# facebookresearch/vggsfm

Hardware: NVIDIA H100
Metric: BA iterations/sec (higher is better)
Workload: dtype f64

## Files before the change

vggsfm_b200/csrc/ba_lm.h:

```cpp
#pragma once
#include <math.h>
#include <stddef.h>
#include "common.cuh"

namespace vgg {

enum : int {
  SCAL_CAM_QUAD = 0, SCAL_CAM_STEP2 = 1, SCAL_PT_QUAD = 2, SCAL_PT_STEP2 = 3, SCAL_GMAX_C = 4, SCAL_GMAX_P = 5,
  SCAL_PT_FAIL = 6, SCAL_CAM_BAD = 7, SCAL_XNORM_C = 8, SCAL_DOUBLES = 16,
};
enum : int {
  SMALL_COST = 0, SMALL_PT_QUAD = 1, SMALL_PT_STEP2 = 2, SMALL_PT_FAIL = 3, SMALL_GMAX_P = 4, SMALL_XNORM_P = 5,
  SMALL_MODEL_CHANGE = 6, SMALL_VEC = 8,
};
enum : int { INFO_CHOL = 0, INFO_TRSV = 1, INFO_FABRIC = 2, INFO_INTS = 4 };

struct LmRecord {
  double scal[8], small[8], chol_info, trsv_info, xnorm_c, fabric_timeout, cg[5];
  double cost() const { return small[SMALL_COST]; }
  double gmax() const {
    return isnan(scal[SCAL_GMAX_C]) || isnan(scal[SCAL_GMAX_P]) ? NAN : fmax(scal[SCAL_GMAX_C], scal[SCAL_GMAX_P]);
  }
};
#define VGG_REC(field) ((int)(offsetof(LmRecord, field) / sizeof(double)))
enum : int { REC_DOUBLES = 24, REC_DOUBLES_CG = 28, REC_CAP = 32 };

struct Reduced {
  double *S, *rhs, *hdiag, *gvec;
};
inline size_t reduced_doubles(int D, int Dpad) { return (size_t)D * Dpad + 3 * (size_t)Dpad; }
// ... 19 lines not shown
```

vggsfm_b200/csrc/ba_schur.cu:

```cuda
#include <stddef.h>
#include <algorithm>
#include <vector>
#include "ba_lm.h"
#include "ba_obs.h"
#include "common.cuh"
#include "dev_probes.h"
#include "syrk_work.h"

namespace vgg {

__device__ __forceinline__ void ar_add(double* local, double* mc, double v) {
  if (mc) asm volatile("multimem.red.relaxed.sys.global.add.f64 [%0], %1;" ::"l"(mc), "d"(v) : "memory");
  else atomicAdd(local, v);
}
__device__ __forceinline__ void ar_put(double* local, double* mc, double v) {
  if (mc) asm volatile("multimem.red.relaxed.sys.global.add.f64 [%0], %1;" ::"l"(mc), "d"(v) : "memory");
  else *local = v;
}

__global__ void jacobi_scale_points_kernel(int N, const double* __restrict__ H_pp, double* __restrict__ sc_p, int enable) {
  const int n = blockIdx.x * blockDim.x + threadIdx.x;
  if (n >= N) return;
  const double* h = H_pp + (size_t)n * 6;
  sc_p[n * 3 + 0] = enable ? 1.0 / (1.0 + sqrt(h[0])) : 1.0;
// ... 323 lines not shown
    for (int mt = 0; mt < 4; ++mt)
#pragma unroll
      for (int nt = 0; nt < 4; ++nt)
#pragma unroll
        for (int h = 0; h < 4; ++h) {
          const int r = wk.bi * SF_BM + wm * 64 + mt * 16 + g + 8 * (h >> 1);
          const int col = wk.bj * SF_BM + wn * 32 + nt * 8 + 2 * t + (h & 1);
          syrk_red_upper(Cmat, Dpad, r, col, wk.bj, diag, acc[mt][nt][h], mc_off, fd);
        }
  }
}

__global__ void scale_damp_kernel(int D, int Dpad, double* __restrict__ A, const double* __restrict__ rhs,
                                  const double* __restrict__ hdiag, const double* __restrict__ sc,
                                  const uint8_t* __restrict__ pconst, double radius, double min_diag, double max_diag,
                                  double* __restrict__ bvec) {
  const int j = blockIdx.x * blockDim.x + threadIdx.x;
  const int i = blockIdx.y;
  if (j >= D || j > i) return;
  const bool ci = pconst[i] != 0, cj = pconst[j] != 0;
  double v;
  if (ci || cj) {
    v = (i == j) ? 1.0 : 0.0;
  } else {
    v = A[(size_t)i * Dpad + j] * sc[i] * sc[j];
    if (i == j) v += fmin(fmax(hdiag[i] * sc[i] * sc[i], min_diag), max_diag) / radius;
  }
  A[(size_t)i * Dpad + j] = v;
  if (i == j) {
    const double b = ci ? 0.0 : rhs[i] * sc[i];
    bvec[i] = b;
    A[(size_t)D * Dpad + i] = b;
    if (i == 0) A[(size_t)D * Dpad + D] = 1e300;
  }
}

__global__ void cam_step_kernel(int D, const double* __restrict__ dcs, size_t dcs_stride, const double* __restrict__ sc,
                                const double* __restrict__ hdiag, const double* __restrict__ gvec,
                                const uint8_t* __restrict__ pconst, double radius, double min_diag, double max_diag,
                                double* __restrict__ d_c, double* __restrict__ scal) {
  const int i = blockIdx.x * blockDim.x + threadIdx.x;
  double a = 0, b = 0, bad = 0;
  if (i < D) {
    const double x = pconst[i] ? 0.0 : dcs[(size_t)i * dcs_stride];
    const double dc = x * sc[i];
    d_c[i] = dc;
    if (!isfinite(x)) bad = 1.0;
    const double dcc = fmin(fmax(hdiag[i] * sc[i] * sc[i], min_diag), max_diag);
    a = pconst[i] ? 0.0 : (x * x * dcc / radius - dc * gvec[i]);
    b = dc * dc;
  }
  a = warp_sum(a); b = warp_sum(b); bad = warp_sum(bad);
  if ((threadIdx.x & 31) == 0) {
    atomicAdd(&scal[SCAL_CAM_QUAD], a);
    atomicAdd(&scal[SCAL_CAM_STEP2], b);
    if (bad > 0) atomicAdd(&scal[SCAL_CAM_BAD], bad);
  }
}

constexpr int BS_W = 16;
template <int MODEL, int MODE, bool ROBUST>
__global__ void __launch_bounds__(BS_W * 32) backsub_kernel(
    int S, int N, const float* __restrict__ uv, const uint8_t* __restrict__ mask, const double* __restrict__ poses,
    const double* __restrict__ intr, const double* __restrict__ points, const uint8_t* __restrict__ point_const,
    const double* __restrict__ d_c, double* __restrict__ wacc, const int* __restrict__ fg_tracks, BaLoss loss) {
  using C = BlkCfg<MODEL, MODE>;
  constexpr int DC = C::DC, NS = C::NS;
  __shared__ double s_cam[BS_W][16];
  __shared__ double s_acc[3][BS_W][32];
  const int lane = threadIdx.x & 31, warp = threadIdx.x >> 5, nw = blockDim.x >> 5;
  const int nlo = blockIdx.x * 32, nhi = min(N, nlo + 32);
// ... 73 lines not shown
    const double s0 = sc_p[n * 3], s1 = sc_p[n * 3 + 1], s2 = sc_p[n * 3 + 2];
    const double e0 = d0 / s0, e1 = d1 / s1, e2 = d2 / s2;
    a = pc ? 0.0 : (e0 * e0 * dpp[n * 3] + e1 * e1 * dpp[n * 3 + 1] + e2 * e2 * dpp[n * 3 + 2]) / radius -
                       (d0 * g0 + d1 * g1 + d2 * g2);
    b = pc ? 0.0 : d0 * d0 + d1 * d1 + d2 * d2;
  }
  a = warp_sum(a); b = warp_sum(b);
  if ((threadIdx.x & 31) == 0) {
    atomicAdd(&scal[SCAL_PT_QUAD], a);
    atomicAdd(&scal[SCAL_PT_STEP2], b);
  }
}

__global__ void cam_update_kernel(int S, int dc, int ns, int model, const double* __restrict__ d_c,
                                  const double* __restrict__ poses, const double* __restrict__ intr,
                                  double* __restrict__ poses_c, double* __restrict__ intr_c) {
  const int s = blockIdx.x * blockDim.x + threadIdx.x;
  if (s >= S) return;
  const double* d = d_c + (size_t)s * dc;
  const double p0 = 2.0 * d[0], p1 = 2.0 * d[1], p2 = 2.0 * d[2];
  const double th2 = p0 * p0 + p1 * p1 + p2 * p2;
  const double th = sqrt(th2);
  double a, b;
  if (th < 1e-12) {
    a = 1.0 - th2 / 6.0;
    b = 0.5 - th2 / 24.0;
  } else {
    a = sin(th) / th;
    b = (1.0 - cos(th)) / th2;
  }
  const bool rot = p0 != 0.0 || p1 != 0.0 || p2 != 0.0;
  double E[9];
// ... 11 lines not shown
  Q[7] = d[4] != 0.0 ? P[7] + d[4] : P[7];
  Q[11] = d[5] != 0.0 ? P[11] + d[5] : P[11];
  const int ni = (model == VGG_SIMPLE_PINHOLE) ? 1 : 2;
  double f = intr[s * 4], k = intr[s * 4 + 3];
  const double* di = dc > 6 ? d + 6 : d_c + (size_t)S * dc;
  if (dc > 6 || ns > 0) {
    if (di[0] != 0.0) f += di[0];
    if (ni > 1 && di[1] != 0.0) k += di[1];
  }
  intr_c[s * 4] = f;
  intr_c[s * 4 + 1] = intr[s * 4 + 1];
  intr_c[s * 4 + 2] = intr[s * 4 + 2];
  intr_c[s * 4 + 3] = k;
}

__global__ void extract_gvec_kernel(int S, int dc, int ns, int KR, const double* __restrict__ camrec,
                                    const double* __restrict__ shared_in, double* __restrict__ gvec) {
  const int i = blockIdx.x * blockDim.x + threadIdx.x;
  const int D = S * dc + ns;
  if (i >= D) return;
  gvec[i] = (i < S * dc) ? camrec[(size_t)(i / dc) * KR + (i % dc)] : shared_in[i - S * dc];
}

__global__ void gradmax_kernel(int D, int N, const double* __restrict__ gvec, const uint8_t* __restrict__ pconst,
                               const double* __restrict__ g_p, const uint8_t* __restrict__ point_const,
                               double* __restrict__ scal) {
  const int i = blockIdx.x * blockDim.x + threadIdx.x;
  unsigned long long mc = 0, mp = 0;
  if (i < D && !pconst[i]) mc = (unsigned long long)__double_as_longlong(fabs(gvec[i]));
  if (i < N * 3 && !(point_const && point_const[i / 3])) mp = (unsigned long long)__double_as_longlong(fabs(g_p[i]));
#pragma unroll
  for (int off = 16; off >= 1; off >>= 1) {
    mc = max(mc, __shfl_xor_sync(0xffffffffu, mc, off));
    mp = max(mp, __shfl_xor_sync(0xffffffffu, mp, off));
  }
  if ((threadIdx.x & 31) == 0) {
// ... 75 lines not shown
    if (!work.empty())
      VGG_CUDA_CHECK(cudaMemcpy(hs.work_dev, work.data(), sizeof(SyrkWork) * work.size(), cudaMemcpyHostToDevice));
    hs.nwork = (int)work.size();
    hs.dev = dev;
    hs.Kpad = Kpad;
    hs.Dpad = Dpad;
    hs.ranges = ranges;
  }
  if (hs.nwork == 0) return VGG_OK;
  syrk_f64_kernel<<<std::min(hs.sms, hs.nwork), SF_THREADS, SF_SMEM_BYTES, st>>>(hs.work_dev, hs.nwork, Kpad, Dpad, Zt, Cmat,
                                                                               mc_off, fd);
  VGG_LAUNCH_CHECK();
  return VGG_OK;
}
int launch_scale_damp(int D, int Dpad, double* A, const double* rhs, const double* hdiag, const double* sc,
                      const uint8_t* pconst, double radius, double min_diag, double max_diag, double* bvec,
                      cudaStream_t st) {
  dim3 grid((D + 255) / 256, D);
  scale_damp_kernel<<<grid, 256, 0, st>>>(D, Dpad, A, rhs, hdiag, sc, pconst, radius, min_diag, max_diag, bvec);
  VGG_LAUNCH_CHECK();
  return VGG_OK;
}
int launch_cam_step(int D, const double* dcs, size_t dcs_stride, const double* sc, const double* hdiag, const double* gvec,
                    const uint8_t* pconst, double radius, double min_diag, double max_diag, double* d_c, double* scal,
                    cudaStream_t st) {
  cam_step_kernel<<<(D + 255) / 256, 256, 0, st>>>(D, dcs, dcs_stride, sc, hdiag, gvec, pconst, radius, min_diag, max_diag, d_c, scal);
  VGG_LAUNCH_CHECK();
  return VGG_OK;
}
int launch_backsub(const vgg_ba_problem* p, const double* d_c, double* wacc, const int* fg_tracks, cudaStream_t st) {
  VGG_PICK_BA_KERNEL(kern, backsub_kernel, p);
  const int nw = std::min(BS_W, p->S);
  kern<<<(p->N + 31) / 32, nw * 32, 0, st>>>(p->S, p->N, p->uv, p->mask, p->poses, p->intr, p->points, p->point_const,
                                             d_c, wacc, fg_tracks, ba_loss_of(p));
  VGG_LAUNCH_CHECK();
  return VGG_OK;
}
int launch_point_step(int N, const double* M, const double* g_p, const double* wacc, const double* sc_p,
                      const double* dpp, const uint8_t* point_const, const double* X, double radius, double* Xc,
                      double* scal, cudaStream_t st) {
  point_step_kernel<<<(N + 127) / 128, 128, 0, st>>>(N, M, g_p, wacc, sc_p, dpp, point_const, X, radius, Xc, scal);
  VGG_LAUNCH_CHECK();
  return VGG_OK;
}
int launch_cam_update(int S, int dc, int ns, int model, const double* d_c, const double* poses, const double* intr,
                      double* poses_c, double* intr_c, cudaStream_t st) {
  cam_update_kernel<<<(S + 127) / 128, 128, 0, st>>>(S, dc, ns, model, d_c, poses, intr, poses_c, intr_c);
  VGG_LAUNCH_CHECK();
  return VGG_OK;
}
int launch_extract_gvec(int S, int dc, int ns, int KR, const double* camrec, const double* shared_in, double* gvec,
                        cudaStream_t st) {
  const int D = S * dc + ns;
  extract_gvec_kernel<<<(D + 255) / 256, 256, 0, st>>>(S, dc, ns, KR, camrec, shared_in, gvec);
  VGG_LAUNCH_CHECK();
  return VGG_OK;
}
int launch_gradmax(int D, int N, const double* gvec, const uint8_t* pconst, const double* g_p,
                   const uint8_t* point_const, double* scal, cudaStream_t st) {
  const int n = D > N * 3 ? D : N * 3;
  gradmax_kernel<<<(n + 255) / 256, 256, 0, st>>>(D, N, gvec, pconst, g_p, point_const, scal);
  VGG_LAUNCH_CHECK();
  return VGG_OK;
}

}

extern "C" {

// ... 35 lines not shown
```

vggsfm_b200/csrc/ba_solve.cu:

```cuda
#include <cublas_v2.h>
#include <math.h>
#include <stdlib.h>
#include <string.h>
#include <map>
#include <vector>
#include "ba_lm.h"
#include "ba_pcg.h"
#include "common.cuh"
#include "dev_probes.h"

namespace vgg {

static thread_local char g_err[512] = "";
thread_local long long g_launch_count = 0;
void set_error(const char* fmt, ...) {
  va_list ap;
  va_start(ap, fmt);
  vsnprintf(g_err, sizeof(g_err), fmt, ap);
  va_end(ap);
}

int ba_build_blocks(const vgg_ba_problem* p, double* cost, double* camrec, double* g_p, double* H_pp, double* W,
                    double* shared_out, int tracks_per_warp, const int* fg_tracks, cudaStream_t stream,
                    bool outputs_zeroed = false);
int launch_jacobi_scale_points(int N, const double* H_pp, double* sc_p, int enable, cudaStream_t st);
int launch_jacobi_scale_cams(int D, const double* hdiag, double* sc_c, int enable, cudaStream_t st);
int launch_point_prep(int N, const double* H_pp, const double* g_p, const double* sc_p, const uint8_t* point_const,
                      double radius, double min_diag, double max_diag, double* M, double* q, double* dpp,
                      double* scal, cudaStream_t st);
int launch_assemble_hc(int S, int dc, int ns, int KR, int Dpad, const double* camrec, const double* shared_in,
                       double* Sraw, double* rhs, double* hdiag, double* gvec, ptrdiff_t mc_off, cudaStream_t st);
int launch_z_build(const vgg_ba_problem* p, int Dpad, const double* M, const double* q, double* Zt, double* rhs,
                   ptrdiff_t mc_off, const int* fg_tracks, cudaStream_t st);
int launch_syrk(int Kpad, int Dpad, const double* Zt, double* Cmat, ptrdiff_t mc_off, const std::vector<int>& kb_ranges,
                const FabricDev& fd, cudaStream_t st);
int launch_scale_damp(int D, int Dpad, double* A, const double* rhs, const double* hdiag, const double* sc,
                      const uint8_t* pconst, double radius, double min_diag, double max_diag, double* bvec,
                      cudaStream_t st);
int launch_cam_step(int D, const double* dcs, size_t dcs_stride, const double* sc, const double* hdiag, const double* gvec,
                    const uint8_t* pconst, double radius, double min_diag, double max_diag, double* d_c, double* scal,
                    cudaStream_t st);
int launch_backsub(const vgg_ba_problem* p, const double* d_c, double* wacc, const int* fg_tracks, cudaStream_t st);
int launch_point_step(int N, const double* M, const double* g_p, const double* wacc, const double* sc_p,
                      const double* dpp, const uint8_t* point_const, const double* X, double radius, double* Xc,
                      double* scal, cudaStream_t st);
int launch_cam_update(int S, int dc, int ns, int model, const double* d_c, const double* poses, const double* intr,
                      double* poses_c, double* intr_c, cudaStream_t st);
int launch_extract_gvec(int S, int dc, int ns, int KR, const double* camrec, const double* shared_in, double* gvec,
                        cudaStream_t st);
int launch_gradmax(int D, int N, const double* gvec, const uint8_t* pconst, const double* g_p,
                   const uint8_t* point_const, double* scal, cudaStream_t st);

int launch_trsv_upper(int n, int lda, const double* A, const double* y, size_t y_stride, double* x, long long* stamps,
                      cudaStream_t st);
size_t chol_workspace_doubles(int n);
int chol_lower_inplace(int n, int lda, double* A, double* Ldiag, int* info, const std::vector<int>& end_blk,
                       int arrow_blk, cudaStream_t st);
int launch_fabric_barrier(const FabricDev& fd, size_t flags_off, unsigned long long epoch, int* err, cudaStream_t st);
int launch_fabric_gather(const FabricDev& fd, int nrows, int nmat, int ncols_vec, int lda, cudaStream_t st);
int launch_fabric_allreduce(const FabricDev& fd, size_t flags_off, size_t mail_off, int mail_len, int parity,
                            unsigned long long epoch, double* vec, int count, int max_slot, int* err, cudaStream_t st);

__global__ void pack_scalars_kernel(const double* __restrict__ scal, const double* __restrict__ small,
// ... 646 lines not shown
  const cudaStream_t st = c.ranks.st;
  int rc;
  const size_t off = fab ? (size_t)(it & 1) * fab->lay.arc : 0;
  const Reduced R = reduced_view(fab ? fab->ar_local + off : L.AR, D, L.Dpad);
  const FabricDev fd = fab ? fab->at(off) : FabricDev{};
  if ((rc = schur_build(L, R, pcur, b, c.band, fd, radius, c.opt.min_lm_diagonal, c.opt.max_lm_diagonal, st, fab)))
    return rc;
  if ((rc = fab ? launch_fabric_gather(fd, D + 3, D + 1, D, L.Dpad, st) : c.ranks.sum(R.S, reduced_doubles(D, L.Dpad))))
    return rc;
  if (first && (rc = launch_jacobi_scale_cams(D, R.hdiag, L.sc_c, c.opt.jacobi_scaling, st))) return rc;
  if ((rc = launch_scale_damp(D, L.Dpad, R.S, R.rhs, R.hdiag, L.sc_c, pcur.param_const, radius, c.opt.min_lm_diagonal,
                              c.opt.max_lm_diagonal, L.bvec, st)))
    return rc;
  if ((rc = chol_lower_inplace(D + 1, L.Dpad, R.S, L.chol_diag, L.dev_info + INFO_CHOL, c.band.end_blk, c.band.arrow_blk, st)))
    return rc;
  VGG_CUDA_CHECK(cudaMemsetAsync(L.dev_info + INFO_TRSV, 0, sizeof(int), st));
  *out = LinStep{L.bvec, R.hdiag, R.gvec, 1};
  if (D <= 7000) return launch_trsv_upper(D, L.Dpad, R.S, R.S + D, (size_t)L.Dpad, L.bvec, nullptr, st);
  cublasHandle_t cb = get_cublas();
  if (!cb || cublasSetStream(cb, st) != CUBLAS_STATUS_SUCCESS) {
    set_error("cublasCreate / cublasSetStream failed");
    return VGG_ESOLVER;
  }
  if (cublasDtrsv(cb, CUBLAS_FILL_MODE_LOWER, CUBLAS_OP_T, CUBLAS_DIAG_NON_UNIT, D, R.S, L.Dpad, R.S + D, L.Dpad) !=
      CUBLAS_STATUS_SUCCESS) {
    set_error("cublasDtrsv failed to launch");
    return VGG_ESOLVER;
  }
  g_launch_count += 1;
  *out = LinStep{R.S + D, R.hdiag, R.gvec, (size_t)L.Dpad};
  return VGG_OK;
// ... 18 lines not shown
    op.camrec = B.camrec;
    op.shared_in = B.shared;
  }
  if (first && (rc = launch_jacobi_scale_cams(L.D, B.hdiag, L.sc_c, c.opt.jacobi_scaling, st))) return rc;
  if ((rc = launch_pcg_init(op, B, L.bvec, st)) || (rc = pcg_run(op, lin, B, L.bvec, c.ranks, st))) return rc;
  *out = LinStep{B.x, B.hdiag, B.gvec, 1};
  return VGG_OK;
}

static int reduce_candidate(const LmContext& c, const vgg_ba_problem& pcur, int cur, bool iterative) {
  const Layout& L = c.L;
  const BlockSet& bn = L.blk[cur ^ 1];
  const cudaStream_t st = c.ranks.st;
  const size_t count = SMALL_VEC + (size_t)L.Dpad;
  int rc;
  VGG_CUDA_CHECK(cudaMemsetAsync(L.small, 0, sizeof(double) * count, st));
  if (iterative && (rc = launch_pcg_model_change(&pcur, L.M, L.blk[cur].g_p, L.wacc, L.d_c, c.band.dev.fg_tracks,
                                                 L.small + SMALL_MODEL_CHANGE, st)))
    return rc;
  VGG_CUDA_CHECK(cudaMemcpyAsync(L.small + SMALL_COST, bn.cost, sizeof(double), cudaMemcpyDeviceToDevice, st));
  VGG_CUDA_CHECK(cudaMemcpyAsync(L.small + SMALL_PT_QUAD, L.scal + SCAL_PT_QUAD, sizeof(double) * 2, cudaMemcpyDeviceToDevice, st));
  VGG_CUDA_CHECK(cudaMemcpyAsync(L.small + SMALL_PT_FAIL, L.scal + SCAL_PT_FAIL, sizeof(double), cudaMemcpyDeviceToDevice, st));
  if ((rc = launch_extract_gvec(L.S, L.dc, L.ns, L.KR, bn.camrec, bn.shared, L.small + SMALL_VEC, st))) return rc;
  if (c.opt.parameter_tolerance > 0.0) {
    xnorm_kernel<<<1, 1024, 0, st>>>(L.S, L.N, L.dc, L.ns, pcur.camera_model, pcur.param_const, pcur.point_const,
                                      pcur.poses, pcur.intr, pcur.points, L.scal + SCAL_XNORM_C, L.small + SMALL_XNORM_P);
    VGG_LAUNCH_CHECK();
  }
  return c.ranks.candidate(L.small, count, L.scal, [&] {
    return launch_gradmax(L.D, L.N, L.small + SMALL_VEC, pcur.param_const, bn.g_p, pcur.point_const, L.scal, st);
  });
}

struct LmState {
  double cost, radius, decrease_factor;
  int invalid_steps;
};

// ... 96 lines not shown
  int cur = 0;
  VGG_CUDA_CHECK(cudaMemcpyAsync(L.poses[0], prob->poses, sizeof(double) * (size_t)S * 12, cudaMemcpyDeviceToDevice, st));
  VGG_CUDA_CHECK(cudaMemcpyAsync(L.intr[0], prob->intr, sizeof(double) * (size_t)S * 4, cudaMemcpyDeviceToDevice, st));
  VGG_CUDA_CHECK(cudaMemcpyAsync(L.points[0], prob->points, sizeof(double) * (size_t)N * 3, cudaMemcpyDeviceToDevice, st));
  if (!lin) VGG_CUDA_CHECK(cudaMemsetAsync(L.Zt, 0, sizeof(double) * (size_t)L.Kpad * L.Dpad, st));
  if (lin) VGG_CUDA_CHECK(cudaMemsetAsync(L.pcg.rhs, 0, sizeof(double) * L.pcg.red_doubles, st));
  VGG_CUDA_CHECK(cudaMemsetAsync(L.d_c, 0, sizeof(double) * L.Dpad, st));

  auto state = [&](int which) {
    vgg_ba_problem p = *prob;
    p.poses = L.poses[which];
    p.intr = L.intr[which];
    p.points = L.points[which];
    return p;
  };
  auto eval = [&](int which) -> int {
    const vgg_ba_problem p = state(which);
    const BlockSet& b = L.blk[which];
    const size_t acc_bytes = reinterpret_cast<char*>(b.H_pp + (size_t)N * 6) - reinterpret_cast<char*>(b.cost);
    VGG_CUDA_CHECK(cudaMemsetAsync(b.cost, 0, acc_bytes, st));
    return ba_build_blocks(&p, b.cost, b.camrec, b.g_p, b.H_pp, nullptr, b.shared, 0, band.dev.fg_tracks, st, true);
  };
  double* h_rec = pinned_scalars();
  if (!h_rec) return VGG_ECUDA;
  const LmRecord& rec = *reinterpret_cast<const LmRecord*>(h_rec);
  VGG_CUDA_CHECK(cudaMemsetAsync(L.dev_info, 0, sizeof(int) * INFO_INTS, st));
  auto read_record = [&]() -> int {
    pack_scalars_kernel<<<1, 32, 0, st>>>(L.scal, L.small, L.dev_info, L.pcg.cg, L.packed);
    VGG_LAUNCH_CHECK();
    VGG_CUDA_CHECK(cudaMemcpyAsync(h_rec, L.packed, sizeof(double) * (lin ? REC_DOUBLES_CG : REC_DOUBLES),
                                   cudaMemcpyDeviceToHost, st));
    VGG_CUDA_CHECK(cudaStreamSynchronize(st));
    if (rec.fabric_timeout != 0.0) {
      set_error("fabric barrier timed out: a peer rank did not arrive");
      return VGG_ECUDA;
    }
    return VGG_OK;
  };

  const BlockSet& b0 = L.blk[cur];
  if ((rc = eval(cur))) return rc;
  if ((rc = launch_jacobi_scale_points(N, b0.H_pp, L.sc_p, opt.jacobi_scaling, st))) return rc;
  VGG_CUDA_CHECK(cudaMemsetAsync(L.small, 0, sizeof(double) * small_count, st));
  VGG_CUDA_CHECK(cudaMemcpyAsync(L.small + SMALL_COST, b0.cost, sizeof(double), cudaMemcpyDeviceToDevice, st));
  if ((rc = launch_extract_gvec(S, L.dc, L.ns, L.KR, b0.camrec, b0.shared, L.small + SMALL_VEC, st))) return rc;
  if ((rc = ranks.sum(L.small, small_count))) return rc;
  VGG_CUDA_CHECK(cudaMemsetAsync(L.scal + SCAL_GMAX_C, 0, sizeof(double) * 2, st));
  if ((rc = launch_gradmax(D, N, L.small + SMALL_VEC, prob->param_const, b0.g_p, prob->point_const, L.scal, st)) ||
      (rc = ranks.max(L.scal + SCAL_GMAX_P)) || (rc = read_record()))
    return rc;

  LmState s{rec.cost(), opt.initial_trust_region_radius, 2.0, 0};
  memset(summary, 0, sizeof(*summary));
  summary->initial_cost = s.cost;
  summary->termination = rec.gmax() <= opt.gradient_tolerance ? VGG_BA_CONVERGENCE_GRADIENT : VGG_BA_NO_CONVERGENCE;
  int it = 0;
  bool have_scale_c = false;

  while (summary->termination == VGG_BA_NO_CONVERGENCE) {
    if (it >= opt.max_num_iterations) break;
// ... 4 lines not shown
    ++it;
    const int cand = cur ^ 1;
    VGG_CUDA_CHECK(cudaMemsetAsync(L.scal, 0, sizeof(double) * SCAL_DOUBLES, st));
    const vgg_ba_problem pcur = state(cur);
    LinStep ls;
    if ((rc = lin ? iterative_step(c, *lin, pcur, L.blk[cur], s.radius, !have_scale_c, &ls)
                  : direct_step(c, pcur, L.blk[cur], it, s.radius, !have_scale_c, &ls)))
      return rc;
    have_scale_c = true;
    if ((rc = launch_cam_step(D, ls.dcs, ls.stride, L.sc_c, ls.hdiag, ls.gvec, prob->param_const, s.radius,
                              opt.min_lm_diagonal, opt.max_lm_diagonal, L.d_c, L.scal, st)) ||
        (rc = launch_backsub(&pcur, L.d_c, L.wacc, band.dev.fg_tracks, st)) ||
        (rc = launch_point_step(N, L.M, L.blk[cur].g_p, L.wacc, L.sc_p, L.dpp, prob->point_const, L.points[cur],
                                s.radius, L.points[cand], L.scal, st)) ||
        (rc = launch_cam_update(S, L.dc, L.ns, prob->camera_model, L.d_c, L.poses[cur], L.intr[cur], L.poses[cand],
                                L.intr[cand], st)) ||
        (rc = eval(cand)) || (rc = reduce_candidate(c, pcur, cur, lin != nullptr)) || (rc = read_record()))
      return rc;
    if (lm_decide(rec, opt, lin != nullptr, it, &s, summary, trace, cg_trace)) cur = cand;
  }

  VGG_CUDA_CHECK(cudaMemcpyAsync(prob->poses, L.poses[cur], sizeof(double) * (size_t)S * 12, cudaMemcpyDeviceToDevice, st));
  VGG_CUDA_CHECK(cudaMemcpyAsync(prob->intr, L.intr[cur], sizeof(double) * (size_t)S * 4, cudaMemcpyDeviceToDevice, st));
  VGG_CUDA_CHECK(cudaMemcpyAsync(prob->points, L.points[cur], sizeof(double) * (size_t)N * 3, cudaMemcpyDeviceToDevice, st));
  VGG_CUDA_CHECK(cudaEventRecord(ev1, st));
  VGG_CUDA_CHECK(cudaEventSynchronize(ev1));
  float ms = 0;
  VGG_CUDA_CHECK(cudaEventElapsedTime(&ms, ev0, ev1));
  summary->iterations = it;
  summary->final_cost = s.cost;
  summary->final_radius = s.radius;
  summary->device_ms = ms;
// ... 93 lines not shown
```

vggsfm_b200/csrc/trsv.cu:

```cuda
#include "common.cuh"
#include "dev_probes.h"

namespace vgg {

namespace {

constexpr int TS_NB = 64;
constexpr int TS_THREADS = 256;
constexpr unsigned long long TS_SENTINEL = 0xffffffffffffffffull;

__global__ void __launch_bounds__(TS_THREADS, 1)
    trsv_upper_kernel(int n, int lda, const double* __restrict__ A, const double* __restrict__ y, size_t y_stride,
                      double* __restrict__ x, long long* __restrict__ stamps) {
  extern __shared__ __align__(16) double ts_smem[];
  double(*Ud)[TS_NB + 1] = reinterpret_cast<double(*)[TS_NB + 1]>(ts_smem);
  double(*Vi)[TS_NB + 1] = reinterpret_cast<double(*)[TS_NB + 1]>(ts_smem + TS_NB * (TS_NB + 1));
  double* xs = ts_smem + 2 * TS_NB * (TS_NB + 1);
  double* accs = xs + TS_NB;
  const int nb = gridDim.x;
  const int b = nb - 1 - (int)blockIdx.x;
  const int r0 = b * TS_NB;
  const int rows = min(TS_NB, n - r0);
  const int tid = threadIdx.x;
  const int r = tid >> 2, seg = tid & 3;
  auto stamp = [&](int k) {
    if (stamps && tid == 0) {
      long long t;
      asm volatile("mov.u64 %0, %%globaltimer;" : "=l"(t));
      stamps[6 * b + k] = t;
    }
  };
  stamp(0);
  double y_mine = 0.0;
  if (tid < TS_NB && tid < rows) y_mine = __ldcg(&y[(size_t)(r0 + tid) * y_stride]);

  for (int e = tid; e < TS_NB * TS_NB; e += TS_THREADS) {
    const int i = e / TS_NB, j = e % TS_NB;
    double v = (i == j) ? 1.0 : 0.0;
    if (i < rows && j < rows && j >= i) v = A[(size_t)(r0 + i) * lda + r0 + j];
    Ud[i][j] = v;
  }
  __syncthreads();
  stamp(1);
  if (tid < TS_NB) xs[tid] = 1.0 / Ud[tid][tid];
  __syncthreads();
  {
    const int c = tid >> 2, part = tid & 3;
    for (int i = TS_NB - 1; i >= 0; --i) {
      double s = 0.0;
      if (i < c) {
        for (int k = i + 1 + part; k <= c; k += 4) s = fma(-Ud[i][k], Vi[k][c], s);
      }
      s += __shfl_xor_sync(0xffffffffu, s, 1);
      s += __shfl_xor_sync(0xffffffffu, s, 2);
      if (part == 0) Vi[i][c] = i > c ? 0.0 : (i == c ? xs[i] : s * xs[i]);
      __syncwarp();
    }
  }
  __syncthreads();
  stamp(2);
  if (tid < TS_NB) accs[tid] = y_mine;
  __syncthreads();
  stamp(5);

  double t0[16], t1[16], t2[16];
  auto load_tile = [&](double (&tile)[16], int j) {
    const int c0 = j * TS_NB + seg * 16;
    const double* src = A + (size_t)(r0 + (r < rows ? r : 0)) * lda + c0;
#pragma unroll
    for (int k = 0; k < 16; ++k) tile[k] = (j > b && r < rows && c0 + k < n) ? src[k] : 0.0;
  };
  double acc = 0.0;
  auto hop = [&](const double (&tile)[16], int j) {
    if (tid < TS_NB) {
      double v = 0.0;
      if (j * TS_NB + tid < n) {
        const volatile unsigned long long* src = reinterpret_cast<const volatile unsigned long long*>(&x[j * TS_NB + tid]);
        unsigned long long bits;
        do {
          bits = *src;
        } while (bits == TS_SENTINEL);
        v = __longlong_as_double((long long)bits);
      }
      xs[tid] = v;
    }
    __syncthreads();
    double s0 = 0.0, s1 = 0.0, s2 = 0.0, s3 = 0.0;
#pragma unroll
    for (int k = 0; k < 16; k += 4) {
      s0 = fma(tile[k], xs[seg * 16 + k], s0);
      s1 = fma(tile[k + 1], xs[seg * 16 + k + 1], s1);
      s2 = fma(tile[k + 2], xs[seg * 16 + k + 2], s2);
      s3 = fma(tile[k + 3], xs[seg * 16 + k + 3], s3);
    }
    acc += (s0 + s1) + (s2 + s3);
    __syncthreads();
  };
  int j = nb - 1;
  if (b < nb - 1) {
  load_tile(t0, j);
  load_tile(t1, j - 1);
  load_tile(t2, j - 2);
  while (j > b) {
    hop(t0, j);
    load_tile(t0, j - 3);
    if (--j <= b) break;
    hop(t1, j);
    load_tile(t1, j - 3);
    if (--j <= b) break;
    hop(t2, j);
    load_tile(t2, j - 3);
    --j;
  }
  }
  stamp(3);
  acc += __shfl_xor_sync(0xffffffffu, acc, 1);
  acc += __shfl_xor_sync(0xffffffffu, acc, 2);
  if (seg == 0) accs[r] -= acc;
  __syncthreads();
  {
    double q0 = 0.0, q1 = 0.0, q2 = 0.0, q3 = 0.0;
#pragma unroll
    for (int k = 0; k < 16; k += 4) {
      const int c = seg * 16 + k;
      q0 = fma(c >= r ? Vi[r][c] : 0.0, accs[c], q0);
      q1 = fma(c + 1 >= r ? Vi[r][c + 1] : 0.0, accs[c + 1], q1);
      q2 = fma(c + 2 >= r ? Vi[r][c + 2] : 0.0, accs[c + 2], q2);
      q3 = fma(c + 3 >= r ? Vi[r][c + 3] : 0.0, accs[c + 3], q3);
    }
    double s = (q0 + q1) + (q2 + q3);
    s += __shfl_xor_sync(0xffffffffu, s, 1);
    s += __shfl_xor_sync(0xffffffffu, s, 2);
    if (seg == 0 && r < rows) {
      unsigned long long bits = (unsigned long long)__double_as_longlong(s);
      if (s != s) bits = 0x7ff8000000000000ull;
      *reinterpret_cast<volatile unsigned long long*>(&x[r0 + r]) = bits;
    }
  }
  if (stamps) {
    __syncthreads();
    stamp(4);
  }
}

}

int launch_trsv_upper(int n, int lda, const double* A, const double* y, size_t y_stride, double* x, long long* stamps,
                      cudaStream_t st) {
  const int nb = (n + TS_NB - 1) / TS_NB;
  VGG_REQUIRE(nb <= 120, "trsv_upper: n too large for one co-resident wave");
  const size_t smem = sizeof(double) * (2 * TS_NB * (TS_NB + 1) + 2 * TS_NB);
  static bool attr = false;
  if (!attr) {
    VGG_CUDA_CHECK(cudaFuncSetAttribute(trsv_upper_kernel, cudaFuncAttributeMaxDynamicSharedMemorySize, (int)smem));
    attr = true;
  }
  VGG_CUDA_CHECK(cudaMemsetAsync(x, 0xFF, sizeof(double) * (size_t)n, st));
  trsv_upper_kernel<<<nb, TS_THREADS, smem, st>>>(n, lda, A, y, y_stride, x, stamps);
  VGG_LAUNCH_CHECK();
  return VGG_OK;
}

}

extern "C" int vgg_dev_trsv_probe(int n, int lda, const double* A_dev, const double* y_dev, size_t y_stride, double* x_dev,
                                  long long* stamps_host) {
  using namespace vgg;
  VGG_REQUIRE(n > 0 && lda >= n && A_dev && y_dev && x_dev && y_stride > 0, "bad argument");
  const int nb = (n + TS_NB - 1) / TS_NB;
  static long long* d = nullptr;
  static int d_cap = 0;
  if (stamps_host && d_cap < 6 * nb) {
    if (d) cudaFree(d);
    VGG_CUDA_CHECK(cudaMalloc(&d, sizeof(long long) * 6 * nb));
    d_cap = 6 * nb;
  }
  if (stamps_host) VGG_CUDA_CHECK(cudaMemset(d, 0, sizeof(long long) * 6 * nb));
  const int rc = launch_trsv_upper(n, lda, A_dev, y_dev, y_stride, x_dev, stamps_host ? d : nullptr, 0);
  if (rc) return rc;
  VGG_CUDA_CHECK(cudaDeviceSynchronize());
  if (stamps_host) VGG_CUDA_CHECK(cudaMemcpy(stamps_host, d, sizeof(long long) * 6 * nb, cudaMemcpyDeviceToHost));
  return VGG_OK;
}
```

Before: 372.8.

## Fold memsets and copies into kernels and widen TRSV blocks to two tiles

Several cudaMemsetAsync and cudaMemcpyAsync calls in the LM loop are removed. The sentinel fill of x moves into scale_damp, zeroing of the candidate accumulator moves into cam_update, and the small-vector assembly (cost, point scalars, gvec) is folded into one extract_gvec launch. cam_step becomes a single block that reduces in shared memory and writes its results instead of using atomics. The TRSV kernel now handles 128 rows per block split into two 64-row halves, with double2 tile loads, which halves the serial block chain; it uses more shared memory and reworks the sentinel handshake.

```diff
diff --git a/vggsfm_b200/csrc/ba_lm.h b/vggsfm_b200/csrc/ba_lm.h
--- a/vggsfm_b200/csrc/ba_lm.h
+++ b/vggsfm_b200/csrc/ba_lm.h
@@ -14,6 +14,7 @@
   SMALL_MODEL_CHANGE = 6, SMALL_VEC = 8,
 };
 enum : int { INFO_CHOL = 0, INFO_TRSV = 1, INFO_FABRIC = 2, INFO_INTS = 4 };
+constexpr unsigned long long TRSV_SENTINEL = 0xffffffffffffffffull;
 
 struct LmRecord {
   double scal[8], small[8], chol_info, trsv_info, xnorm_c, fabric_timeout, cg[5];
diff --git a/vggsfm_b200/csrc/ba_schur.cu b/vggsfm_b200/csrc/ba_schur.cu
--- a/vggsfm_b200/csrc/ba_schur.cu
+++ b/vggsfm_b200/csrc/ba_schur.cu
@@ -361,7 +361,7 @@
 __global__ void scale_damp_kernel(int D, int Dpad, double* __restrict__ A, const double* __restrict__ rhs,
                                   const double* __restrict__ hdiag, const double* __restrict__ sc,
                                   const uint8_t* __restrict__ pconst, double radius, double min_diag, double max_diag,
-                                  double* __restrict__ bvec) {
+                                  double* __restrict__ x) {
   const int j = blockIdx.x * blockDim.x + threadIdx.x;
   const int i = blockIdx.y;
   if (j >= D || j > i) return;
@@ -376,32 +376,46 @@
   A[(size_t)i * Dpad + j] = v;
   if (i == j) {
     const double b = ci ? 0.0 : rhs[i] * sc[i];
-    bvec[i] = b;
+    x[i] = __longlong_as_double((long long)TRSV_SENTINEL);
     A[(size_t)D * Dpad + i] = b;
     if (i == 0) A[(size_t)D * Dpad + D] = 1e300;
   }
 }
 
-__global__ void cam_step_kernel(int D, const double* __restrict__ dcs, size_t dcs_stride, const double* __restrict__ sc,
-                                const double* __restrict__ hdiag, const double* __restrict__ gvec,
-                                const uint8_t* __restrict__ pconst, double radius, double min_diag, double max_diag,
-                                double* __restrict__ d_c, double* __restrict__ scal) {
-  const int i = blockIdx.x * blockDim.x + threadIdx.x;
+constexpr int CS_THREADS = 1024;
+__global__ void __launch_bounds__(CS_THREADS) cam_step_kernel(
+    int D, const double* __restrict__ dcs, size_t dcs_stride, const double* __restrict__ sc,
+    const double* __restrict__ hdiag, const double* __restrict__ gvec, const uint8_t* __restrict__ pconst,
+    double radius, double min_diag, double max_diag, double* __restrict__ d_c, double* __restrict__ scal) {
+  __shared__ double red[3][CS_THREADS / 32];
   double a = 0, b = 0, bad = 0;
-  if (i < D) {
+  for (int i = threadIdx.x; i < D; i += CS_THREADS) {
     const double x = pconst[i] ? 0.0 : dcs[(size_t)i * dcs_stride];
     const double dc = x * sc[i];
     d_c[i] = dc;
-    if (!isfinite(x)) bad = 1.0;
+    if (!isfinite(x)) bad += 1.0;
     const double dcc = fmin(fmax(hdiag[i] * sc[i] * sc[i], min_diag), max_diag);
-    a = pconst[i] ? 0.0 : (x * x * dcc / radius - dc * gvec[i]);
-    b = dc * dc;
+    a += pconst[i] ? 0.0 : (x * x * dcc / radius - dc * gvec[i]);
+    b += dc * dc;
   }
   a = warp_sum(a); b = warp_sum(b); bad = warp_sum(bad);
+  const int w = threadIdx.x >> 5;
   if ((threadIdx.x & 31) == 0) {
-    atomicAdd(&scal[SCAL_CAM_QUAD], a);
-    atomicAdd(&scal[SCAL_CAM_STEP2], b);
-    if (bad > 0) atomicAdd(&scal[SCAL_CAM_BAD], bad);
+    red[0][w] = a;
+    red[1][w] = b;
+    red[2][w] = bad;
+  }
+  __syncthreads();
+  if (threadIdx.x == 0) {
+    a = b = bad = 0.0;
+    for (int k = 0; k < CS_THREADS / 32; ++k) {
+      a += red[0][k];
+      b += red[1][k];
+      bad += red[2][k];
+    }
+    scal[SCAL_CAM_QUAD] = a;
+    scal[SCAL_CAM_STEP2] = b;
+    scal[SCAL_CAM_BAD] = bad;
   }
 }
 
@@ -505,8 +519,10 @@
 
 __global__ void cam_update_kernel(int S, int dc, int ns, int model, const double* __restrict__ d_c,
                                   const double* __restrict__ poses, const double* __restrict__ intr,
-                                  double* __restrict__ poses_c, double* __restrict__ intr_c) {
+                                  double* __restrict__ poses_c, double* __restrict__ intr_c, double* __restrict__ acc,
+                                  size_t acc_count) {
   const int s = blockIdx.x * blockDim.x + threadIdx.x;
+  for (size_t k = s; k < acc_count; k += (size_t)gridDim.x * blockDim.x) acc[k] = 0.0;
   if (s >= S) return;
   const double* d = d_c + (size_t)s * dc;
   const double p0 = 2.0 * d[0], p1 = 2.0 * d[1], p2 = 2.0 * d[2];
@@ -548,12 +564,22 @@
   intr_c[s * 4 + 3] = k;
 }
 
-__global__ void extract_gvec_kernel(int S, int dc, int ns, int KR, const double* __restrict__ camrec,
-                                    const double* __restrict__ shared_in, double* __restrict__ gvec) {
+__global__ void extract_gvec_kernel(int S, int dc, int ns, int KR, int Dpad, const double* __restrict__ camrec,
+                                    const double* __restrict__ shared_in, const double* __restrict__ cost,
+                                    const double* __restrict__ scal, double* __restrict__ small) {
   const int i = blockIdx.x * blockDim.x + threadIdx.x;
   const int D = S * dc + ns;
-  if (i >= D) return;
-  gvec[i] = (i < S * dc) ? camrec[(size_t)(i / dc) * KR + (i % dc)] : shared_in[i - S * dc];
+  if (i >= SMALL_VEC + Dpad) return;
+  double v = 0.0;
+  if (i >= SMALL_VEC) {
+    const int k = i - SMALL_VEC;
+    if (k < D) v = (k < S * dc) ? camrec[(size_t)(k / dc) * KR + (k % dc)] : shared_in[k - S * dc];
+  } else if (i == SMALL_COST) {
+    v = *cost;
+  } else if (scal && (i == SMALL_PT_QUAD || i == SMALL_PT_STEP2 || i == SMALL_PT_FAIL)) {
+    v = scal[i == SMALL_PT_QUAD ? SCAL_PT_QUAD : i == SMALL_PT_STEP2 ? SCAL_PT_STEP2 : SCAL_PT_FAIL];
+  }
+  small[i] = v;
 }
 
 __global__ void gradmax_kernel(int D, int N, const double* __restrict__ gvec, const uint8_t* __restrict__ pconst,
@@ -659,17 +685,18 @@
   return VGG_OK;
 }
 int launch_scale_damp(int D, int Dpad, double* A, const double* rhs, const double* hdiag, const double* sc,
-                      const uint8_t* pconst, double radius, double min_diag, double max_diag, double* bvec,
+                      const uint8_t* pconst, double radius, double min_diag, double max_diag, double* x,
                       cudaStream_t st) {
   dim3 grid((D + 255) / 256, D);
-  scale_damp_kernel<<<grid, 256, 0, st>>>(D, Dpad, A, rhs, hdiag, sc, pconst, radius, min_diag, max_diag, bvec);
+  scale_damp_kernel<<<grid, 256, 0, st>>>(D, Dpad, A, rhs, hdiag, sc, pconst, radius, min_diag, max_diag, x);
   VGG_LAUNCH_CHECK();
   return VGG_OK;
 }
 int launch_cam_step(int D, const double* dcs, size_t dcs_stride, const double* sc, const double* hdiag, const double* gvec,
                     const uint8_t* pconst, double radius, double min_diag, double max_diag, double* d_c, double* scal,
                     cudaStream_t st) {
-  cam_step_kernel<<<(D + 255) / 256, 256, 0, st>>>(D, dcs, dcs_stride, sc, hdiag, gvec, pconst, radius, min_diag, max_diag, d_c, scal);
+  cam_step_kernel<<<1, CS_THREADS, 0, st>>>(D, dcs, dcs_stride, sc, hdiag, gvec, pconst, radius, min_diag, max_diag, d_c,
+                                           scal);
   VGG_LAUNCH_CHECK();
   return VGG_OK;
 }
@@ -689,15 +716,17 @@
   return VGG_OK;
 }
 int launch_cam_update(int S, int dc, int ns, int model, const double* d_c, const double* poses, const double* intr,
-                      double* poses_c, double* intr_c, cudaStream_t st) {
-  cam_update_kernel<<<(S + 127) / 128, 128, 0, st>>>(S, dc, ns, model, d_c, poses, intr, poses_c, intr_c);
-  VGG_LAUNCH_CHECK();
-  return VGG_OK;
-}
-int launch_extract_gvec(int S, int dc, int ns, int KR, const double* camrec, const double* shared_in, double* gvec,
-                        cudaStream_t st) {
-  const int D = S * dc + ns;
-  extract_gvec_kernel<<<(D + 255) / 256, 256, 0, st>>>(S, dc, ns, KR, camrec, shared_in, gvec);
+                      double* poses_c, double* intr_c, double* acc, size_t acc_count, cudaStream_t st) {
+  const size_t threads = std::max<size_t>((size_t)S, std::min<size_t>(acc_count, (size_t)128 * 512));
+  cam_update_kernel<<<(unsigned)((threads + 127) / 128), 128, 0, st>>>(S, dc, ns, model, d_c, poses, intr, poses_c,
+                                                                        intr_c, acc, acc_count);
+  VGG_LAUNCH_CHECK();
+  return VGG_OK;
+}
+int launch_extract_gvec(int S, int dc, int ns, int KR, int Dpad, const double* camrec, const double* shared_in,
+                        const double* cost, const double* scal, double* small, cudaStream_t st) {
+  extract_gvec_kernel<<<(SMALL_VEC + Dpad + 255) / 256, 256, 0, st>>>(S, dc, ns, KR, Dpad, camrec, shared_in, cost, scal,
+                                                                       small);
   VGG_LAUNCH_CHECK();
   return VGG_OK;
 }
diff --git a/vggsfm_b200/csrc/ba_solve.cu b/vggsfm_b200/csrc/ba_solve.cu
--- a/vggsfm_b200/csrc/ba_solve.cu
+++ b/vggsfm_b200/csrc/ba_solve.cu
@@ -35,7 +35,7 @@
 int launch_syrk(int Kpad, int Dpad, const double* Zt, double* Cmat, ptrdiff_t mc_off, const std::vector<int>& kb_ranges,
                 const FabricDev& fd, cudaStream_t st);
 int launch_scale_damp(int D, int Dpad, double* A, const double* rhs, const double* hdiag, const double* sc,
-                      const uint8_t* pconst, double radius, double min_diag, double max_diag, double* bvec,
+                      const uint8_t* pconst, double radius, double min_diag, double max_diag, double* x,
                       cudaStream_t st);
 int launch_cam_step(int D, const double* dcs, size_t dcs_stride, const double* sc, const double* hdiag, const double* gvec,
                     const uint8_t* pconst, double radius, double min_diag, double max_diag, double* d_c, double* scal,
@@ -45,8 +45,9 @@
                       const double* dpp, const uint8_t* point_const, const double* X, double radius, double* Xc,
                       double* scal, cudaStream_t st);
 int launch_cam_update(int S, int dc, int ns, int model, const double* d_c, const double* poses, const double* intr,
-                      double* poses_c, double* intr_c, cudaStream_t st);
-int launch_extract_gvec(int S, int dc, int ns, int KR, const double* camrec, const double* shared_in, double* gvec,
+                      double* poses_c, double* intr_c, double* acc, size_t acc_count, cudaStream_t st);
+int launch_extract_gvec(int S, int dc, int ns, int KR, int Dpad, const double* camrec, const double* shared_in,
+                        const double* cost, const double* scal, double* small,
                         cudaStream_t st);
 int launch_gradmax(int D, int N, const double* gvec, const uint8_t* pconst, const double* g_p,
                    const uint8_t* point_const, double* scal, cudaStream_t st);
@@ -723,7 +724,6 @@
     return rc;
   if ((rc = chol_lower_inplace(D + 1, L.Dpad, R.S, L.chol_diag, L.dev_info + INFO_CHOL, c.band.end_blk, c.band.arrow_blk, st)))
     return rc;
-  VGG_CUDA_CHECK(cudaMemsetAsync(L.dev_info + INFO_TRSV, 0, sizeof(int), st));
   *out = LinStep{L.bvec, R.hdiag, R.gvec, 1};
   if (D <= 7000) return launch_trsv_upper(D, L.Dpad, R.S, R.S + D, (size_t)L.Dpad, L.bvec, nullptr, st);
   cublasHandle_t cb = get_cublas();
@@ -772,14 +772,11 @@
   const cudaStream_t st = c.ranks.st;
   const size_t count = SMALL_VEC + (size_t)L.Dpad;
   int rc;
-  VGG_CUDA_CHECK(cudaMemsetAsync(L.small, 0, sizeof(double) * count, st));
+  if ((rc = launch_extract_gvec(L.S, L.dc, L.ns, L.KR, L.Dpad, bn.camrec, bn.shared, bn.cost, L.scal, L.small, st)))
+    return rc;
   if (iterative && (rc = launch_pcg_model_change(&pcur, L.M, L.blk[cur].g_p, L.wacc, L.d_c, c.band.dev.fg_tracks,
                                                  L.small + SMALL_MODEL_CHANGE, st)))
     return rc;
-  VGG_CUDA_CHECK(cudaMemcpyAsync(L.small + SMALL_COST, bn.cost, sizeof(double), cudaMemcpyDeviceToDevice, st));
-  VGG_CUDA_CHECK(cudaMemcpyAsync(L.small + SMALL_PT_QUAD, L.scal + SCAL_PT_QUAD, sizeof(double) * 2, cudaMemcpyDeviceToDevice, st));
-  VGG_CUDA_CHECK(cudaMemcpyAsync(L.small + SMALL_PT_FAIL, L.scal + SCAL_PT_FAIL, sizeof(double), cudaMemcpyDeviceToDevice, st));
-  if ((rc = launch_extract_gvec(L.S, L.dc, L.ns, L.KR, bn.camrec, bn.shared, L.small + SMALL_VEC, st))) return rc;
   if (c.opt.parameter_tolerance > 0.0) {
     xnorm_kernel<<<1, 1024, 0, st>>>(L.S, L.N, L.dc, L.ns, pcur.camera_model, pcur.param_const, pcur.point_const,
                                       pcur.poses, pcur.intr, pcur.points, L.scal + SCAL_XNORM_C, L.small + SMALL_XNORM_P);
@@ -906,11 +903,14 @@
     p.points = L.points[which];
     return p;
   };
-  auto eval = [&](int which) -> int {
+  auto acc_doubles = [&](int which) {
+    const BlockSet& b = L.blk[which];
+    return (size_t)(b.H_pp + (size_t)N * 6 - b.cost);
+  };
+  auto eval = [&](int which, bool zeroed) -> int {
     const vgg_ba_problem p = state(which);
     const BlockSet& b = L.blk[which];
-    const size_t acc_bytes = reinterpret_cast<char*>(b.H_pp + (size_t)N * 6) - reinterpret_cast<char*>(b.cost);
-    VGG_CUDA_CHECK(cudaMemsetAsync(b.cost, 0, acc_bytes, st));
+    if (!zeroed) VGG_CUDA_CHECK(cudaMemsetAsync(b.cost, 0, sizeof(double) * acc_doubles(which), st));
     return ba_build_blocks(&p, b.cost, b.camrec, b.g_p, b.H_pp, nullptr, b.shared, 0, band.dev.fg_tracks, st, true);
   };
   double* h_rec = pinned_scalars();
@@ -931,11 +931,10 @@
   };
 
   const BlockSet& b0 = L.blk[cur];
-  if ((rc = eval(cur))) return rc;
+  if ((rc = eval(cur, false))) return rc;
   if ((rc = launch_jacobi_scale_points(N, b0.H_pp, L.sc_p, opt.jacobi_scaling, st))) return rc;
-  VGG_CUDA_CHECK(cudaMemsetAsync(L.small, 0, sizeof(double) * small_count, st));
-  VGG_CUDA_CHECK(cudaMemcpyAsync(L.small + SMALL_COST, b0.cost, sizeof(double), cudaMemcpyDeviceToDevice, st));
-  if ((rc = launch_extract_gvec(S, L.dc, L.ns, L.KR, b0.camrec, b0.shared, L.small + SMALL_VEC, st))) return rc;
+  if ((rc = launch_extract_gvec(S, L.dc, L.ns, L.KR, L.Dpad, b0.camrec, b0.shared, b0.cost, nullptr, L.small, st)))
+    return rc;
   if ((rc = ranks.sum(L.small, small_count))) return rc;
   VGG_CUDA_CHECK(cudaMemsetAsync(L.scal + SCAL_GMAX_C, 0, sizeof(double) * 2, st));
   if ((rc = launch_gradmax(D, N, L.small + SMALL_VEC, prob->param_const, b0.g_p, prob->point_const, L.scal, st)) ||
@@ -970,8 +969,8 @@
         (rc = launch_point_step(N, L.M, L.blk[cur].g_p, L.wacc, L.sc_p, L.dpp, prob->point_const, L.points[cur],
                                 s.radius, L.points[cand], L.scal, st)) ||
         (rc = launch_cam_update(S, L.dc, L.ns, prob->camera_model, L.d_c, L.poses[cur], L.intr[cur], L.poses[cand],
-                                L.intr[cand], st)) ||
-        (rc = eval(cand)) || (rc = reduce_candidate(c, pcur, cur, lin != nullptr)) || (rc = read_record()))
+                                L.intr[cand], L.blk[cand].cost, acc_doubles(cand), st)) ||
+        (rc = eval(cand, true)) || (rc = reduce_candidate(c, pcur, cur, lin != nullptr)) || (rc = read_record()))
       return rc;
     if (lm_decide(rec, opt, lin != nullptr, it, &s, summary, trace, cg_trace)) cur = cand;
   }
diff --git a/vggsfm_b200/csrc/trsv.cu b/vggsfm_b200/csrc/trsv.cu
--- a/vggsfm_b200/csrc/trsv.cu
+++ b/vggsfm_b200/csrc/trsv.cu
@@ -1,3 +1,4 @@
+#include "ba_lm.h"
 #include "common.cuh"
 #include "dev_probes.h"
 
@@ -6,72 +7,114 @@
 namespace {
 
 constexpr int TS_NB = 64;
-constexpr int TS_THREADS = 256;
-constexpr unsigned long long TS_SENTINEL = 0xffffffffffffffffull;
+constexpr int TS_ROWS = 2 * TS_NB;
+constexpr int TS_THREADS = 4 * TS_ROWS;
+constexpr int TS_STAMPS = 7;
+
+__device__ __forceinline__ void half_sync(int half) {
+  if (half == 0) asm volatile("bar.sync 1, %0;" ::"n"(TS_THREADS / 2) : "memory");
+  else asm volatile("bar.sync 2, %0;" ::"n"(TS_THREADS / 2) : "memory");
+}
 
 __global__ void __launch_bounds__(TS_THREADS, 1)
     trsv_upper_kernel(int n, int lda, const double* __restrict__ A, const double* __restrict__ y, size_t y_stride,
                       double* __restrict__ x, long long* __restrict__ stamps) {
   extern __shared__ __align__(16) double ts_smem[];
-  double(*Ud)[TS_NB + 1] = reinterpret_cast<double(*)[TS_NB + 1]>(ts_smem);
-  double(*Vi)[TS_NB + 1] = reinterpret_cast<double(*)[TS_NB + 1]>(ts_smem + TS_NB * (TS_NB + 1));
-  double* xs = ts_smem + 2 * TS_NB * (TS_NB + 1);
-  double* accs = xs + TS_NB;
+  double(*Ud)[TS_NB][TS_NB + 1] = reinterpret_cast<double(*)[TS_NB][TS_NB + 1]>(ts_smem);
+  double(*Vi)[TS_NB][TS_NB + 1] = reinterpret_cast<double(*)[TS_NB][TS_NB + 1]>(ts_smem + 3 * TS_NB * (TS_NB + 1));
+  double* xs = ts_smem + 5 * TS_NB * (TS_NB + 1);
+  double* accs = xs + TS_ROWS;
   const int nb = gridDim.x;
+  const int nb64 = (n + TS_NB - 1) / TS_NB;
   const int b = nb - 1 - (int)blockIdx.x;
-  const int r0 = b * TS_NB;
-  const int rows = min(TS_NB, n - r0);
+  const int r0 = b * TS_ROWS;
+  const int rows = min(TS_ROWS, n - r0);
   const int tid = threadIdx.x;
   const int r = tid >> 2, seg = tid & 3;
+  const int half = r / TS_NB;
+  const int jb = 2 * b + 1;
+  __shared__ long long stamp_s[TS_STAMPS];
   auto stamp = [&](int k) {
     if (stamps && tid == 0) {
       long long t;
       asm volatile("mov.u64 %0, %%globaltimer;" : "=l"(t));
-      stamps[6 * b + k] = t;
+      stamp_s[k] = t;
     }
   };
   stamp(0);
   double y_mine = 0.0;
-  if (tid < TS_NB && tid < rows) y_mine = __ldcg(&y[(size_t)(r0 + tid) * y_stride]);
-
-  for (int e = tid; e < TS_NB * TS_NB; e += TS_THREADS) {
-    const int i = e / TS_NB, j = e % TS_NB;
-    double v = (i == j) ? 1.0 : 0.0;
-    if (i < rows && j < rows && j >= i) v = A[(size_t)(r0 + i) * lda + r0 + j];
-    Ud[i][j] = v;
+  if (tid < TS_ROWS && tid < rows) y_mine = __ldcg(&y[(size_t)(r0 + tid) * y_stride]);
+
+  auto load_tile = [&](double2 (&tile)[8], int j, bool ok) {
+    const int c0 = j * TS_NB + 2 * seg;
+    const double* src = A + (size_t)(r0 + (r < rows ? r : 0)) * lda + c0;
+    ok = ok && r < rows;
+#pragma unroll
+    for (int m = 0; m < 8; ++m) {
+      const int c = c0 + 8 * m;
+      if (ok && c + 1 < n) {
+        tile[m] = *reinterpret_cast<const double2*>(src + 8 * m);
+      } else {
+        tile[m].x = (ok && c < n) ? src[8 * m] : 0.0;
+        tile[m].y = 0.0;
+      }
+    }
+  };
+  for (int e = tid; e < 3 * TS_NB * TS_NB; e += TS_THREADS) {
+    const int h = e / (TS_NB * TS_NB), i = (e / TS_NB) % TS_NB, j = e % TS_NB;
+    const int hc = h ? 1 : 0;
+    const int hr = min(TS_NB, max(0, rows - hc * TS_NB)), o = r0 + hc * TS_NB;
+    double v;
+    if (h < 2) {
+      v = (i == j) ? 1.0 : 0.0;
+      if (i < hr && j < hr && j >= i) v = A[(size_t)(o + i) * lda + o + j];
+    } else {
+      v = (i < min(TS_NB, rows) && j < hr) ? A[(size_t)(r0 + i) * lda + o + j] : 0.0;
+    }
+    Ud[h][i][j] = v;
   }
   __syncthreads();
   stamp(1);
-  if (tid < TS_NB) xs[tid] = 1.0 / Ud[tid][tid];
+  if (tid < TS_ROWS) xs[tid] = 1.0 / Ud[tid / TS_NB][tid % TS_NB][tid % TS_NB];
   __syncthreads();
   {
-    const int c = tid >> 2, part = tid & 3;
+    const int c = r % TS_NB, part = seg;
+    double(*U)[TS_NB + 1] = Ud[half];
+    double(*V)[TS_NB + 1] = Vi[half];
+    const double* piv = xs + half * TS_NB;
     for (int i = TS_NB - 1; i >= 0; --i) {
       double s = 0.0;
       if (i < c) {
-        for (int k = i + 1 + part; k <= c; k += 4) s = fma(-Ud[i][k], Vi[k][c], s);
+        for (int k = i + 1 + part; k <= c; k += 4) s = fma(-U[i][k], V[k][c], s);
       }
       s += __shfl_xor_sync(0xffffffffu, s, 1);
       s += __shfl_xor_sync(0xffffffffu, s, 2);
-      if (part == 0) Vi[i][c] = i > c ? 0.0 : (i == c ? xs[i] : s * xs[i]);
+      if (part == 0) V[i][c] = i > c ? 0.0 : (i == c ? piv[i] : s * piv[i]);
       __syncwarp();
     }
   }
   __syncthreads();
   stamp(2);
-  if (tid < TS_NB) accs[tid] = y_mine;
+  if (tid < TS_ROWS) accs[tid] = y_mine;
   __syncthreads();
   stamp(5);
 
-  double t0[16], t1[16], t2[16];
-  auto load_tile = [&](double (&tile)[16], int j) {
-    const int c0 = j * TS_NB + seg * 16;
-    const double* src = A + (size_t)(r0 + (r < rows ? r : 0)) * lda + c0;
-#pragma unroll
-    for (int k = 0; k < 16; ++k) tile[k] = (j > b && r < rows && c0 + k < n) ? src[k] : 0.0;
-  };
+  double2 t0[8], t1[8], t2[8];
   double acc = 0.0;
-  auto hop = [&](const double (&tile)[16], int j) {
+  auto matvec = [&](const double2 (&tile)[8], int xo) {
+    double s0 = 0.0, s1 = 0.0, s2 = 0.0, s3 = 0.0;
+#pragma unroll
+    for (int m = 0; m < 8; m += 2) {
+      const double2 xa = *reinterpret_cast<const double2*>(xs + xo + 8 * m + 2 * seg);
+      const double2 xb = *reinterpret_cast<const double2*>(xs + xo + 8 * (m + 1) + 2 * seg);
+      s0 = fma(tile[m].x, xa.x, s0);
+      s1 = fma(tile[m].y, xa.y, s1);
+      s2 = fma(tile[m + 1].x, xb.x, s2);
+      s3 = fma(tile[m + 1].y, xb.y, s3);
+    }
+    acc += (s0 + s1) + (s2 + s3);
+  };
+  auto hop = [&](const double2 (&tile)[8], int j) {
     if (tid < TS_NB) {
       double v = 0.0;
       if (j * TS_NB + tid < n) {
@@ -79,67 +122,75 @@
         unsigned long long bits;
         do {
           bits = *src;
-        } while (bits == TS_SENTINEL);
+        } while (bits == TRSV_SENTINEL);
         v = __longlong_as_double((long long)bits);
       }
       xs[tid] = v;
     }
     __syncthreads();
-    double s0 = 0.0, s1 = 0.0, s2 = 0.0, s3 = 0.0;
-#pragma unroll
-    for (int k = 0; k < 16; k += 4) {
-      s0 = fma(tile[k], xs[seg * 16 + k], s0);
-      s1 = fma(tile[k + 1], xs[seg * 16 + k + 1], s1);
-      s2 = fma(tile[k + 2], xs[seg * 16 + k + 2], s2);
-      s3 = fma(tile[k + 3], xs[seg * 16 + k + 3], s3);
-    }
-    acc += (s0 + s1) + (s2 + s3);
+    matvec(tile, 0);
     __syncthreads();
   };
-  int j = nb - 1;
-  if (b < nb - 1) {
-  load_tile(t0, j);
-  load_tile(t1, j - 1);
-  load_tile(t2, j - 2);
-  while (j > b) {
+  int j = nb64 - 1;
+  if (j > jb) {
+  load_tile(t0, j, true);
+  load_tile(t1, j - 1, j - 1 > jb);
+  load_tile(t2, j - 2, j - 2 > jb);
+  while (j > jb) {
     hop(t0, j);
-    load_tile(t0, j - 3);
-    if (--j <= b) break;
+    load_tile(t0, j - 3, j - 3 > jb);
+    if (--j <= jb) break;
     hop(t1, j);
-    load_tile(t1, j - 3);
-    if (--j <= b) break;
+    load_tile(t1, j - 3, j - 3 > jb);
+    if (--j <= jb) break;
     hop(t2, j);
-    load_tile(t2, j - 3);
+    load_tile(t2, j - 3, j - 3 > jb);
     --j;
   }
   }
   stamp(3);
-  acc += __shfl_xor_sync(0xffffffffu, acc, 1);
-  acc += __shfl_xor_sync(0xffffffffu, acc, 2);
-  if (seg == 0) accs[r] -= acc;
-  __syncthreads();
-  {
+  auto solve_half = [&]() {
+    const int rr = r % TS_NB, o = half * TS_NB;
+    acc += __shfl_xor_sync(0xffffffffu, acc, 1);
+    acc += __shfl_xor_sync(0xffffffffu, acc, 2);
+    if (seg == 0) accs[r] -= acc;
+    half_sync(half);
     double q0 = 0.0, q1 = 0.0, q2 = 0.0, q3 = 0.0;
 #pragma unroll
     for (int k = 0; k < 16; k += 4) {
       const int c = seg * 16 + k;
-      q0 = fma(c >= r ? Vi[r][c] : 0.0, accs[c], q0);
-      q1 = fma(c + 1 >= r ? Vi[r][c + 1] : 0.0, accs[c + 1], q1);
-      q2 = fma(c + 2 >= r ? Vi[r][c + 2] : 0.0, accs[c + 2], q2);
-      q3 = fma(c + 3 >= r ? Vi[r][c + 3] : 0.0, accs[c + 3], q3);
+      q0 = fma(c >= rr ? Vi[half][rr][c] : 0.0, accs[o + c], q0);
+      q1 = fma(c + 1 >= rr ? Vi[half][rr][c + 1] : 0.0, accs[o + c + 1], q1);
+      q2 = fma(c + 2 >= rr ? Vi[half][rr][c + 2] : 0.0, accs[o + c + 2], q2);
+      q3 = fma(c + 3 >= rr ? Vi[half][rr][c + 3] : 0.0, accs[o + c + 3], q3);
     }
     double s = (q0 + q1) + (q2 + q3);
     s += __shfl_xor_sync(0xffffffffu, s, 1);
     s += __shfl_xor_sync(0xffffffffu, s, 2);
-    if (seg == 0 && r < rows) {
-      unsigned long long bits = (unsigned long long)__double_as_longlong(s);
-      if (s != s) bits = 0x7ff8000000000000ull;
-      *reinterpret_cast<volatile unsigned long long*>(&x[r0 + r]) = bits;
-    }
+    if (seg == 0) {
+      xs[r] = s;
+      if (r < rows) {
+        unsigned long long bits = (unsigned long long)__double_as_longlong(s);
+        if (s != s) bits = 0x7ff8000000000000ull;
+        *reinterpret_cast<volatile unsigned long long*>(&x[r0 + r]) = bits;
+      }
+    }
+  };
+  if (half == 1) solve_half();
+  __syncthreads();
+  stamp(6);
+  if (half == 0) {
+    double2 td[8];
+#pragma unroll
+    for (int m = 0; m < 8; ++m) td[m] = make_double2(Ud[2][r][8 * m + 2 * seg], Ud[2][r][8 * m + 2 * seg + 1]);
+    matvec(td, TS_NB);
+    solve_half();
   }
   if (stamps) {
     __syncthreads();
     stamp(4);
+    if (tid == 0)
+      for (int k = 0; k < TS_STAMPS; ++k) stamps[TS_STAMPS * b + k] = stamp_s[k];
   }
 }
 
@@ -147,15 +198,14 @@
 
 int launch_trsv_upper(int n, int lda, const double* A, const double* y, size_t y_stride, double* x, long long* stamps,
                       cudaStream_t st) {
-  const int nb = (n + TS_NB - 1) / TS_NB;
+  const int nb = (n + TS_ROWS - 1) / TS_ROWS;
   VGG_REQUIRE(nb <= 120, "trsv_upper: n too large for one co-resident wave");
-  const size_t smem = sizeof(double) * (2 * TS_NB * (TS_NB + 1) + 2 * TS_NB);
+  const size_t smem = sizeof(double) * (5 * TS_NB * (TS_NB + 1) + 2 * TS_ROWS);
   static bool attr = false;
   if (!attr) {
     VGG_CUDA_CHECK(cudaFuncSetAttribute(trsv_upper_kernel, cudaFuncAttributeMaxDynamicSharedMemorySize, (int)smem));
     attr = true;
   }
-  VGG_CUDA_CHECK(cudaMemsetAsync(x, 0xFF, sizeof(double) * (size_t)n, st));
   trsv_upper_kernel<<<nb, TS_THREADS, smem, st>>>(n, lda, A, y, y_stride, x, stamps);
   VGG_LAUNCH_CHECK();
   return VGG_OK;
@@ -167,18 +217,20 @@
                                   long long* stamps_host) {
   using namespace vgg;
   VGG_REQUIRE(n > 0 && lda >= n && A_dev && y_dev && x_dev && y_stride > 0, "bad argument");
-  const int nb = (n + TS_NB - 1) / TS_NB;
+  const int nb = (n + TS_ROWS - 1) / TS_ROWS;
   static long long* d = nullptr;
   static int d_cap = 0;
-  if (stamps_host && d_cap < 6 * nb) {
+  if (stamps_host && d_cap < TS_STAMPS * nb) {
     if (d) cudaFree(d);
-    VGG_CUDA_CHECK(cudaMalloc(&d, sizeof(long long) * 6 * nb));
-    d_cap = 6 * nb;
-  }
-  if (stamps_host) VGG_CUDA_CHECK(cudaMemset(d, 0, sizeof(long long) * 6 * nb));
+    VGG_CUDA_CHECK(cudaMalloc(&d, sizeof(long long) * TS_STAMPS * nb));
+    d_cap = TS_STAMPS * nb;
+  }
+  if (stamps_host) VGG_CUDA_CHECK(cudaMemset(d, 0, sizeof(long long) * TS_STAMPS * nb));
+  static_assert(TRSV_SENTINEL == ~0ull, "the fill below writes all-ones bytes");
+  VGG_CUDA_CHECK(cudaMemsetAsync(x_dev, 0xFF, sizeof(double) * (size_t)n, 0));
   const int rc = launch_trsv_upper(n, lda, A_dev, y_dev, y_stride, x_dev, stamps_host ? d : nullptr, 0);
   if (rc) return rc;
   VGG_CUDA_CHECK(cudaDeviceSynchronize());
-  if (stamps_host) VGG_CUDA_CHECK(cudaMemcpy(stamps_host, d, sizeof(long long) * 6 * nb, cudaMemcpyDeviceToHost));
+  if (stamps_host) VGG_CUDA_CHECK(cudaMemcpy(stamps_host, d, sizeof(long long) * TS_STAMPS * nb, cudaMemcpyDeviceToHost));
   return VGG_OK;
 }
```

Measured after the change: 379.4 (median of 6 runs). +1.8%, better.
